# RemyMuj/UnityRayTracer

Measured on AMD Instinct MI355X. Metric: Mrays/sec @1920x1080, 8 bounces, higher is better.
Workload: dtype f32

## Files before the change

### include/urt_math.h

```cpp
#pragma once
#include <stdint.h>

#if defined(__HIPCC__)
#include <hip/hip_runtime.h>
#define URT_HD __host__ __device__ __forceinline__
#else
#define URT_HD inline __attribute__((always_inline))
#endif

#if defined(__clang__)
#pragma clang fp contract(off)
#endif

namespace urt {

static constexpr float kPI        = 3.14159265f;
static constexpr float kEPSILON   = 1e-8f;
static constexpr float kFLOAT_MAX = 3.402823466e+38f;
#define URT_INF (__builtin_inff())

URT_HD float f_fma(float a, float b, float c) { return __builtin_fmaf(a, b, c); }
URT_HD float f_sqrt(float x) { return __builtin_sqrtf(x); }
URT_HD float f_floor(float x) { return __builtin_floorf(x); }
URT_HD float f_abs(float x) { return __builtin_fabsf(x); }
// ... 189 lines not shown
  }
}
URT_HD void cslab(float cx, float cy, float cz, float hx, float hy, float hz, const CRay& R, float tbest, float& tn, float& tf) {
  float mx = f_fma(cx, R.idir.x, R.b.x), my = f_fma(cy, R.idir.y, R.b.y), mz = f_fma(cz, R.idir.z, R.b.z);
  float dx = f_fma(hx, f_abs(R.idir.x), R.pa.x), dy = f_fma(hy, f_abs(R.idir.y), R.pa.y), dz = f_fma(hz, f_abs(R.idir.z), R.pa.z);
  tn = f_max(f_max(f_max(mx - dx, my - dy), mz - dz), 0.0f);
  tf = f_min(f_min(f_min(mx + dx, my + dy), mz + dz), tbest);
}

URT_HD bool tlas_cull(float t_min, float t_max, float t_ground) {
  const float kappa = 0.015625f;
  float s = kappa * (f_abs(t_min) + f_abs(t_max));
  bool miss = (t_min - t_max) > s;
  bool behind = t_max < -s;
  bool beyond = (t_min - t_ground) > kappa * (f_abs(t_min) + f_abs(t_ground));
  return miss || behind || beyond;
}

URT_HD float f_div_const(float x, float c, float y) {
  float ax = f_abs(x);
  if (!(ax >= 1e-30f && ax <= 3.0e38f)) return x / c;
  float q = x * y;
  float r = f_fma(-q, c, x);
  return f_fma(r, y, q);
}

URT_HD float rand_next(float& seed, float px, float py) {
  float a = f_div_const(seed + f_div_const(seed, 17.0f, 1.0f / 17.0f), 100.0f, 1.0f / 100.0f);
  float d = dot2(px, py, 12.9898f, 78.233f);
  float r = f_frac(f_sin(a * d) * 43758.5453f);
  seed = seed + 0.5f;
  return r;
}

}
```

### unityraytracer_amd/csrc/context_impl.h

```cpp
#pragma once
#include <hip/hip_runtime.h>

#include <algorithm>
#include <cmath>
#include <cstdio>
#include <cstring>
#include <new>
#include <string>
#include <unordered_map>
#include <utility>
#include <vector>

#include "../../include/urt.h"
#include "../../include/urt_math.h"
#include "blas_builder.h"
#include "kernels.h"
#include "owned.h"
#include "urt_device.h"

namespace urtd {

struct Buffer {
  int count = 0, stride = 0;
  std::vector<uint8_t> host;
// ... 120 lines not shown
    int32_t* d_mesh_leaf = nullptr;
    size_t cap_mesh_leaf = 0;
    int walk_f4 = 0;
    int n_blas_nodes = 0;
    int n_scene_tris = 0;
    int scene_max_depth = 0;
    int tlas_stack = 2, blas_stack = 2;
    unsigned int watchdog_steps = 1u << 16;
    std::vector<int32_t> h_mesh_root, h_small_first;
    std::vector<int32_t> h_vert_lo, h_vert_hi;
    int n_vertices = 0, n_normals = 0;
    std::vector<float> h_cost_base;
    std::vector<uint8_t> prev_mesh_objects;
  } scene;
  uint64_t scene_epoch = 0;
  float last_prepare_ms = 0;
  int last_builder = 0;
  uint64_t refitted_meshes = 0, incremental_preps = 0;
  uint64_t deformed_meshes = 0, renormed_meshes = 0, deform_bytes = 0, forced_rebuilds = 0;
  float last_cost_ratio = 0;
  urtd::BlasCache blas_cache;
  int sched_groups = 0;
  urtd::DeviceBuf<float4> zero_sky;

  urtd::PathQueues q{};
  urtd::DeviceBuf<float4> q_store[2][4];
  urtd::DeviceBuf<unsigned int> q_counts;

  urtd::DeviceBuf<urtd::DevCounters> d_counters;
  static constexpr size_t kStampOffset = urtd::kWorkShards * 128, kStampBytes = 65536 * 16 * sizeof(unsigned long long), kWorkCounterBytes = kStampOffset + kStampBytes;
  urtd::DeviceBuf<unsigned int> d_next;
  urtd::DeviceBuf<float4> d_mail;
  static constexpr int kTableSlots = 4;
  urtd::PinnedBuf<urtd::FrameUniforms> h_tables; urtd::DeviceBuf<urtd::FrameUniforms> d_tables;
  urtd::Event table_ev[kTableSlots];
  unsigned int table_next = 0;
  uint64_t pixels_dispatched = 0;
  int n_cus = 256;

  uint64_t dispatches = 0;
  std::vector<std::pair<urtd::Event, urtd::Event>> timing;
  float trace_ms = 0;

  enum class OpKind { BlendAdd, BlendHistory, Copy, PackRows };
  struct PostOp {
    OpKind kind;
    int frame;
    urt_handle src = 0, dst = 0;
    float sample = 0;
    urt_handle count = 0; float max_history = 0;
    void* dense = nullptr; int first_row = 0, row_stride = 1; bool rgb = false;
    bool touches(urt_handle t) const { return src == t || dst == t || count == t; }
  };
  struct Pending {
    int n = 0, limit = 1;
    urt_handle tex = 0;
    uint64_t scene_epoch = 0;
    urtd::DevScene S{};
    urtd::FrameParams P{};
    urtd::FrameTable T{};
    int front_mode = 0; bool count = false;
    std::vector<PostOp> ops;
  } pend;
  urtd::DeviceBuf<float4> slab;
  size_t slab_stride = 0;
  int slab_frames = 0;
  urt_handle slab_tex = 0;
// ... 120 lines not shown
```

### unityraytracer_amd/csrc/experiments.h

```cpp
#pragma once

#if defined(URT_STAMPS) || defined(URT_SCHED_OCC) || defined(URT_SERVE_OCC) || defined(URT_SERVE_SLEEP) || defined(URT_SKY_FASTWRAP) || \
    defined(URT_SAH_BINS) || defined(URT_AB)
#ifndef URT_EXPERIMENT
#error "A/B, probe and diagnostic switches (-DURT_STAMPS, -DURT_SCHED_OCC, -DURT_SAH_BINS, ...) need -DURT_EXPERIMENT: the library then reports a negative urt_abi_version and loaders refuse it unless they opt in (csrc/experiments.h)"
#endif
#endif

#ifdef URT_EXPERIMENT
#define URT_ABI_SIGN (-1)
#else
#define URT_ABI_SIGN 1
#endif
```

### unityraytracer_amd/csrc/frame_batch.cpp

```cpp
#include "experiments.h"
#include "context_impl.h"

#include "reproject.h"

namespace urtd {

static unsigned int sched_trip_cap(urt_context* ctx, const FrameParams& P, int n_frames) {
  if (ctx->opt.watchdog_cap > 0) return (unsigned int)ctx->opt.watchdog_cap;
  uint64_t per = std::max<uint64_t>(1, (uint64_t)std::max(1, P.num_rays) * (uint64_t)std::max(1, P.num_bounces) / 8u);
  uint64_t cap = (1ull << 24) * (uint64_t)std::max(1, n_frames) * per;
  return (unsigned int)std::min<uint64_t>(cap, 0xfffffff0ull);
}

static int ensure_queues(urt_context* ctx, size_t n_paths, size_t n_counts) {
  for (int k = 0; k < 8; k++) {
    if (int rc = reserve(ctx, ctx->q_store[k / 4][k % 4], n_paths, "path queue allocation", touch(ctx))) return rc;
    ctx->q.s[k / 4][k % 4] = ctx->q_store[k / 4][k % 4].get();
  }
  if (int rc = reserve(ctx, ctx->q_counts, n_counts, "path queue allocation", touch(ctx))) return rc;
  ctx->q.counts = ctx->q_counts.get();
  return URT_OK;
}

int resolve_timing(urt_context* ctx) {
// ... 157 lines not shown

template <typename Launch>
static int timed_launch(urt_context* ctx, hipStream_t st, int kernel_mode, int front_mode, const FrameParams& P, bool count, int waves_per_cu, Launch launch) {
  Event e0, e1;
  if (ctx->opt.time_dispatch) {
    int rc = take_event(ctx, &e0); if (rc) return rc;
    rc = take_event(ctx, &e1); if (rc) return rc;
    URT_HIP(ctx, hipEventRecord(e0.get(), st));
  }
  TraceLaunchRecord rec{};
  hipError_t le = launch(&rec);
  if (ctx->opt.time_dispatch) {
    (void)hipEventRecord(e1.get(), st);
    ctx->timing.emplace_back(std::move(e0), std::move(e1));
  }
  ctx->launches++;
  if (le != hipSuccess) return fail(ctx, URT_ERR_HIP, std::string("kernel launch: ") + hipGetErrorString(le));
  record_launch(ctx, rec, kernel_mode, front_mode, P, count, waves_per_cu);
  return URT_OK;
}

static constexpr int kAutoFrames = 64;

static int launch_sched_frames(urt_context* ctx, const DevScene& S, const FrameParams& P, const FrameTable& T, float4* result,
                        int front_mode, bool count, hipStream_t st = nullptr, unsigned int* next = nullptr) {
  if (!st) { st = touch(ctx); next = ctx->d_next.get(); }
  if (!ctx->h_tables) {
    URT_HIP(ctx, ctx->h_tables.alloc((size_t)kMaxFramesPerLaunch * urt_context::kTableSlots));
    URT_HIP(ctx, ctx->d_tables.alloc((size_t)kMaxFramesPerLaunch * urt_context::kTableSlots));
    for (Event& ev : ctx->table_ev) URT_HIP(ctx, ev.create(hipEventDisableTiming));
  }
  const unsigned int slot = ctx->table_next++ % (unsigned int)urt_context::kTableSlots;
  if (ctx->table_next > (unsigned int)urt_context::kTableSlots) URT_HIP(ctx, hipEventSynchronize(ctx->table_ev[slot].get()));
  FrameUniforms* h_slot = ctx->h_tables.get() + (size_t)slot * kMaxFramesPerLaunch;
  FrameUniforms* d_table = ctx->d_tables.get() + (size_t)slot * kMaxFramesPerLaunch;
  std::memcpy(h_slot, T.f, sizeof(FrameUniforms) * (size_t)P.n_frames);
  URT_HIP(ctx, hipMemcpyAsync(d_table, h_slot, sizeof(FrameUniforms) * (size_t)P.n_frames, hipMemcpyHostToDevice, st));
  URT_HIP(ctx, hipEventRecord(ctx->table_ev[slot].get(), st));
  int waves_per_block = P.block_threads / 64;
  long want = ((long)P.tiles_x * P.n_strips * P.n_frames + waves_per_block - 1) / waves_per_block;
  int wpc = ctx->opt.waves_per_cu;
  if (wpc <= 0) wpc = P.serve ? 16 : 20;
  if (ctx->sched_groups > 0) wpc = ctx->sched_groups * waves_per_block;
  long resident = (long)ctx->n_cus * wpc / waves_per_block;
  int nb = (int)std::max(1L, std::min(want, resident));
  if (P.serve) {
    if (int rc = reserve(ctx, ctx->d_mail, (size_t)nb * (size_t)P.block_threads * 2, "mailbox allocation", touch(ctx))) return rc;
  }
  int rc = timed_launch(ctx, st, P.serve ? 5 : 3, front_mode, P, count, wpc, [&](TraceLaunchRecord* rec) {
    return P.serve ? launch_serve(S, P, d_table, result, ctx->d_counters.get(), next, ctx->d_mail.get(), nb, front_mode, count, st, rec)
                   : launch_sched(S, P, d_table, result, ctx->d_counters.get(), next, nb, front_mode, count, st, rec);
  });
  if (rc == URT_OK) ctx->last_launch.cones = !P.serve && !count && !S.blas_qnodes && S.blas_cnodes && ctx->scene.cones_in_use ? 1 : 0;
  return rc;
}

struct BlendRun { int frames; urt_handle present; size_t end; };
static BlendRun blend_run(const std::vector<PostOp>& ops, size_t i, urt_handle result_tex, float* samples) {
  const PostOp& op = ops[i];
  size_t j = i, j_present = i;
  int cnt = 0, cnt_present = 0;
  urt_handle present = 0;
  while (j < ops.size() && cnt <= kMaxFramesPerLaunch) {
    const PostOp& q = ops[j];
    if (q.kind == op.kind && q.dst == op.dst && q.count == op.count && q.max_history == op.max_history && q.frame == op.frame + cnt &&
        cnt < kMaxFramesPerLaunch) { samples[cnt++] = q.sample; j++; }
    else if (q.kind == OpKind::Copy && q.src == op.dst && q.dst != op.dst && q.dst != op.count && q.dst != result_tex && (present == 0 || q.dst == present)) {
      present = q.dst; j++; j_present = j; cnt_present = cnt;
    } else break;
  }
// ... 193 lines not shown
  if ((mode == 3 || mode == 5) && P.num_bounces >= (1 << 24)) mode = 2;
  bool count = ctx->opt.count_stats != 0;
  const int region[4] = {P.region_w, P.region_h, first_row, row_stride};
  const bool full_cover = P.region_w == res->w && P.region_h == res->h && first_row == 0 && row_stride == 1;

  if (mode == 3 || mode == 5) {
    bool top_in_front = ctx->opt.top_front < 0 ? S.n_meshes > 1 : ctx->opt.top_front != 0;
    P.serve = mode == 5 && ctx->scene.n_blas_nodes > 0;
    P.pool_inloop = ctx->opt.serve_refill;
    int front_mode = configure_sched(ctx, S, P, top_in_front);
    P.shade_split = ctx->opt.shade_split != 0;
    set_handout(ctx, P);
    P.front_fuse = ctx->opt.front_fuse == 0 ? 0 : (S.n_mesh_tlas == 1 && S.n_meshes > 0 && S.n_spheres == 0 ? 2 : 1);
    const FrameUniforms fu = bound_camera(ctx);
    bool same_region = res->n_regions == 1 && std::memcmp(res->rg, region, sizeof region) == 0;
    bool renamable = !res->external && !res->ptr_exposed && (full_cover || (!res->other_writes && (res->n_regions == 0 || same_region)));
    int limit = renamable ? batch_limit(ctx, P) : 1;
    urt_context::Pending& B = ctx->pend;
    if (B.n > 0) {
      const FrameParams& Q = B.P;
      bool same = B.tex == res_h && B.scene_epoch == ctx->scene_epoch && B.S.sky == S.sky && B.S.sky_w == S.sky_w && B.S.sky_h == S.sky_h &&
                  B.count == count && B.front_mode == front_mode && Q.serve == P.serve && Q.num_bounces == P.num_bounces && Q.num_rays == P.num_rays &&
                  Q.width == P.width && Q.height == P.height && Q.region_w == P.region_w && Q.region_h == P.region_h &&
                  Q.first_group_row == P.first_group_row && Q.row_stride == P.row_stride && B.n < B.limit && limit > 1;
      if (!same) { int rc = flush_pending(ctx); if (rc) return rc; }
    }
    if (limit > 1 && B.n == 0) {
      int rc = ensure_slab(ctx, res_h, *res, limit); if (rc) return rc;
      if (!ctx->slab || ctx->slab_tex != res_h || ctx->slab_frames < 2) limit = 1;
    }
    if (B.n == 0) { int rc = bind_sky(ctx, S); if (rc) return rc; }
    if (limit <= 1) {
      FrameTable T{};
      T.f[0] = fu;
      P.frame_group = 1;
      int rc = launch_sched_frames(ctx, S, P, T, res->dev, front_mode, count);
      if (rc) return rc;
    } else {
      if (B.n == 0) {
        B.limit = std::min(limit, ctx->slab_frames);
        B.tex = res_h; B.scene_epoch = ctx->scene_epoch; B.S = S; B.P = P; B.front_mode = front_mode; B.count = count;
      }
      B.T.f[B.n] = fu;
      res->dev = ctx->slab.get() + (size_t)B.n * ctx->slab_stride;
      B.n++;
    }
  } else {
    int rc = flush_pending(ctx); if (rc) return rc;
    int nb = 0, k = 0;
    if (mode == 1) {
      size_t n_paths = (size_t)P.tiles_x * 64 * (size_t)P.n_strips;
      rc = ensure_queues(ctx, n_paths, (size_t)P.num_rays * (size_t)(P.num_bounces + 1));
      if (rc) return rc;
    } else if (mode == 2) {
      int waves_per_block = P.block_threads / 64;
      long want = ((long)P.tiles_x * P.n_strips + waves_per_block - 1) / waves_per_block;
      int wpc = ctx->opt.waves_per_cu;
      if (wpc <= 0) wpc = 20;
      long resident = (long)ctx->n_cus * wpc / waves_per_block;
      nb = (int)std::max(1L, std::min(want, resident));
    } else if (mode == 4) {
      P.block_threads = 64;
      P.refill_min = ctx->opt.pool_refill; P.blas_min = ctx->opt.pool_blas_min; P.blas_exit = ctx->opt.pool_blas_exit;
      P.pool_inloop = ctx->opt.pool_inloop; P.pool_other_min = ctx->opt.pool_other_min;
      k = ctx->opt.pool_k;
      size_t lds = pool_lds_bytes(P, k);
      while (k > 1 && lds > 160 * 1024) { k--; lds = pool_lds_bytes(P, k); }
      if (lds > 160 * 1024) return fail(ctx, URT_ERR_OUT_OF_MEMORY, "kernel_mode 4: the scene's traversal stacks do not fit the LDS of one CU; use kernel_mode 3");
      int fit = (int)std::max<size_t>(1, (160 * 1024) / lds);
      int wpc = ctx->opt.waves_per_cu > 0 ? ctx->opt.waves_per_cu : fit;
      long want = ((long)P.tiles_x * P.n_strips * 64 + 64L * k - 1) / (64L * k);
      nb = (int)std::max(1L, std::min(want, (long)ctx->n_cus * wpc));
    }
    const hipStream_t st = touch(ctx);
    rc = timed_launch(ctx, st, mode, 0, P, count, ctx->opt.waves_per_cu, [&](TraceLaunchRecord* rec) {
      switch (mode) {
// ... 15 lines not shown
```

### unityraytracer_amd/csrc/frame_device.h

```cpp
#pragma once
#include <hip/hip_runtime.h>
#include <stdint.h>

#include "../../include/urt_math.h"
#include "urt_device.h"
#include "kernels.h"

using namespace urt;
using namespace urtd;

#include "camera_device.h"
#include "trace_device.h"
#include "sky_device.h"
#include "shade_device.h"

namespace {

template <bool COUNT>
__device__ __forceinline__ HitRec trace(const DevScene& S, v3 o, v3 d, int* tl, int* bl, LocalCounters& lc) {
  return trace_ray<COUNT, false>(S, o, d, URT_INF, tl, bl, lc);
}

typedef const __attribute__((address_space(4))) float* kfloatp;
__device__ __forceinline__ kfloatp kernarg_floats(unsigned byte_offset) {
  const __attribute__((address_space(4))) char* p = (const __attribute__((address_space(4))) char*)__builtin_amdgcn_kernarg_segment_ptr();
  p += byte_offset;
  asm volatile("" : "+s"(p));
  return (kfloatp)p;
}

template <unsigned P_OFF>
__device__ __forceinline__ void camera_ray(const FrameParams& P, int x, int y, float& seed, v3& o, v3& d) {
  float u, v;
  jitter_uv(seed, (float)x, (float)y, P.pixel_off_x, P.pixel_off_y, P.width, P.height, u, v);
  kfloatp c2w = kernarg_floats(P_OFF + (unsigned)__builtin_offsetof(FrameParams, c2w));
  kfloatp invp = kernarg_floats(P_OFF + (unsigned)__builtin_offsetof(FrameParams, invp));
  camera_ray_uv(c2w, invp, u, v, o, d);
}
__device__ __forceinline__ void camera_ray_frame(const FrameUniforms* T, int f, const FrameParams& P, int x, int y, bool new_pixel, float& seed, v3& o, v3& d) {
  kfloatp q = (kfloatp)(unsigned long long)(T + __builtin_amdgcn_readfirstlane(f));
  if (new_pixel) seed = q[34];
  float px = (float)x, py = (float)y;
  float r0 = rand_next(seed, px, py);
  float r1 = rand_next(seed, px, py);
  float u = axis_uv(px + r0 + q[32], P.width);
  float v = axis_uv(py + r1 + q[33], P.height);
  camera_ray_uv(q, q + 16, u, v, o, d);
}
static_assert(__builtin_offsetof(FrameUniforms, invp) == 64 && __builtin_offsetof(FrameUniforms, pixel_off_x) == 128 &&
              __builtin_offsetof(FrameUniforms, seed) == 136, "camera_ray_frame indexes the table as floats");

template <typename F>
__device__ __forceinline__ void for_each_frame(bool pred, int frame, F&& body) {
  unsigned long long todo = wballot(pred);
  while (todo) {
    int f = __builtin_amdgcn_readlane(frame, __builtin_ctzll(todo));
    bool mine = pred && frame == f;
    body(f, mine);
    todo &= ~wballot(mine);
  }
}

static constexpr unsigned kPOffAfterScene = (unsigned)((sizeof(DevScene) + alignof(FrameParams) - 1) / alignof(FrameParams) * alignof(FrameParams));

__device__ __forceinline__ bool tile_pixel(const FrameParams& P, int& x, int& y) {
  int wave = threadIdx.x >> 6, lane = threadIdx.x & 63;
  int b = blockIdx.x;
  int G = P.xcd_run;
  int sb = ((b / (8 * G)) * 8 + (b & 7)) * G + ((b >> 3) % G);
  int tile = sb * (blockDim.x >> 6) + wave;
  int ntiles = P.tiles_x * P.n_strips;
  if (tile >= ntiles) return false;
  int ty = tile / P.tiles_x, tx = tile - ty * P.tiles_x;
  x = tx * 8 + (lane & 7);
  y = (P.first_group_row + ty * P.row_stride) * 8 + (lane >> 3);
  return x < P.region_w && y < P.region_h;
}

__device__ __forceinline__ unsigned int wave_sum(unsigned int v) {
  for (int off = 32; off > 0; off >>= 1) v += __shfl_xor(v, off, 64);
  return v;
}

// ... 139 lines not shown
    }
  }
  return run_word(nshard, f, t0, vt * 64u, exh);
}

__device__ __forceinline__ bool wg_fetch_pixels(const FrameParams& P, unsigned long long want, bool mine, unsigned int* next,
                                                unsigned int ntiles, unsigned long long* rs, bool& exhausted, int& x, int& y,
                                                unsigned int tiles_per_frame, int* frame, unsigned long long* n_adds = nullptr) {
  const int lane = threadIdx.x & 63;
  const unsigned int n = (unsigned int)__popcll(want);
  const unsigned int rank = (unsigned int)__popcll(want & ((1ull << lane) - 1ull));
  unsigned int taken = 0;
  bool got = false;
  for (int round = 0; round < 2; round++) {
    unsigned long long s = 0;
    unsigned int k = 0, avail = 0;
    bool fetch = false;
    for (int tries = 0;; tries++) {
      if (tries == kRunCasTries) return got;
      s = wave_uniform64(__hip_atomic_load(rs, __ATOMIC_RELAXED, __HIP_MEMORY_SCOPE_WORKGROUP));
      avail = ((unsigned int)(s >> 11) & 0x7ffu) - ((unsigned int)s & 0x7ffu);
      unsigned long long s2;
      if (avail) {
        k = min(n - taken, avail);
        fetch = k == avail && !(s & kRunExhausted);
        s2 = (s + k) | (fetch ? kRunFetching : 0ull);
      } else if (s & kRunExhausted) { exhausted = true; return got; }
      else if (s & kRunFetching) { if (n == 64u) __builtin_amdgcn_s_sleep(2); return got; }
      else { k = 0; fetch = true; s2 = s | kRunFetching; }
      unsigned long long seen = s;
      if (lane == 0) __hip_atomic_compare_exchange_strong(rs, &seen, s2, __ATOMIC_RELAXED, __ATOMIC_RELAXED, __HIP_MEMORY_SCOPE_WORKGROUP);
      if (wave_uniform64(seen) == s) break;
    }
    if (mine && rank >= taken && rank < taken + k) {
      const unsigned int idx = ((unsigned int)s & 0x7ffu) + (rank - taken);
      unsigned int tile = ((unsigned int)(s >> 24) & 0xffffffu) + (idx >> 6), f = (unsigned int)(s >> 48) & 0x7fu;
      if (tile >= tiles_per_frame) { unsigned int q = tile / tiles_per_frame; f += q; tile -= q * tiles_per_frame; }
      *frame = (int)f;
      if (P.tile_order == 1) tile = tiles_per_frame - 1u - tile;
      got = slot_pixel(P, tile, idx & 63u, x, y);
    }
    taken += k;
    if (!fetch) { if (k == avail) exhausted = true; break; }
    const unsigned long long ns = wg_fetch_run(P, (unsigned int)(s >> 55) & 63u, next, ntiles, tiles_per_frame);
    if (lane == 0) __hip_atomic_store(rs, ns, __ATOMIC_RELAXED, __HIP_MEMORY_SCOPE_WORKGROUP);
    if (n_adds) ++*n_adds;
    if (taken == n) break;
  }
  return got;
}

__device__ __forceinline__ void report_watchdog(const FrameParams& P, DevCounters* shard) {
  atomicAdd(&shard->watchdog, 1ull);
  if (P.trip_flag) __hip_atomic_fetch_add(P.trip_flag, 1u, __ATOMIC_RELAXED, __HIP_MEMORY_SCOPE_SYSTEM);
}

__device__ __forceinline__ void finish_path(const FrameParams& P, float4* result, int pixel, int ray_index, v3 res, float seed) {
  int x = pixel & 0xffff, y = (unsigned)pixel >> 16;
  size_t at = (size_t)y * P.width + x;
  v3 avg = res;
  if (ray_index > 0) { float4 prev = result[at]; avg = xyz(prev) + res; }
  if (ray_index == P.num_rays - 1) {
    float n = (float)P.num_rays;
    result[at] = make_float4(avg.x / n, avg.y / n, avg.z / n, 1.0f);
  } else {
    result[at] = make_float4(avg.x, avg.y, avg.z, seed);
  }
}

}
```

### unityraytracer_amd/csrc/kernels.h

```cpp
#pragma once
#include <hip/hip_runtime.h>
#include "urt_device.h"

namespace urtd {

struct TraceLaunchRecord { char kernel[96]; int n_blocks, block_threads, lds_bytes; };

hipError_t launch_mega(const DevScene& S, const FrameParams& P, float4* result, DevCounters* ctr, bool count, hipStream_t st, TraceLaunchRecord* rec);
hipError_t launch_wavefront(const DevScene& S, const FrameParams& P, const PathQueues& Q, float4* result, DevCounters* ctr,
                            bool count, hipStream_t st, TraceLaunchRecord* rec);
hipError_t launch_persist(const DevScene& S, const FrameParams& P, float4* result, DevCounters* ctr, unsigned int* next,
                          int n_blocks, bool count, hipStream_t st, TraceLaunchRecord* rec);
hipError_t launch_sched(const DevScene& S, const FrameParams& P, const FrameUniforms* T, float4* result, DevCounters* ctr,
                        unsigned int* next, int n_blocks, int front_mode, bool count, hipStream_t st, TraceLaunchRecord* rec);
hipError_t launch_serve(const DevScene& S, const FrameParams& P, const FrameUniforms* T, float4* result, DevCounters* ctr,
                        unsigned int* next, float4* mail, int n_blocks, int front_mode, bool count, hipStream_t st, TraceLaunchRecord* rec);
hipError_t launch_blit_add_multi(const float4* src, size_t frame_stride, int n, const float* samples, float4* dst, float4* present,
                                 size_t n_pixels, hipStream_t st);
size_t sched_lds_bytes(const DevScene& S, const FrameParams& P);
hipError_t launch_pool(const DevScene& S, const FrameParams& P, float4* result, DevCounters* ctr, unsigned int* next,
                       int n_blocks, int k, bool count, hipStream_t st, TraceLaunchRecord* rec);
size_t pool_lds_bytes(const FrameParams& P, int k);
hipError_t launch_blit_add(const float4* src, float4* dst, size_t n_pixels, float sample, hipStream_t st);
hipError_t launch_pack_rows(float4* img, float4* dense, int width, int height, int first_group_row, int row_stride,
                            int n_strips, bool to_dense, hipStream_t st);

hipError_t launch_pack_rows_rgb(float4* img, float* dense, int width, int height, int first_group_row, int row_stride,
                                int n_strips, bool to_dense, float alpha, hipStream_t st);

}
```

### unityraytracer_amd/csrc/kernels.hip

```cpp
#include "experiments.h"
#include "front_device.h"
#include "launch_host.h"
#include <utility>

namespace {

#ifndef URT_SCHED_OCC
#define URT_SCHED_OCC 5
#endif
template <bool COUNT, int BLOCK, int FMODE, bool MULTI, bool QN = false>
__global__ __launch_bounds__(BLOCK, URT_SCHED_OCC) void k_sched(DevScene S, FrameParams P, const FrameUniforms* __restrict__ T, float4* __restrict__ result, DevCounters* ctr,
                                               unsigned int* __restrict__ next) {
  constexpr bool CONES = !COUNT && !QN;
  extern __shared__ int lds[];
  float4* lds4 = (float4*)lds;
  const float4* top = lds4 + 1;
  if (threadIdx.x == 0) *(unsigned long long*)lds = run_word(blockIdx.x & ((unsigned int)P.n_shards - 1u), 0, 0, 0, false);
  for (int i = threadIdx.x; i < P.top_nodes * 4; i += blockDim.x) lds4[1 + i] = S.blas_cnodes[i];
  int at = 1 + P.top_nodes * 4;
  FrontLds L;
  if (P.lds_mesh) {
    for (int i = threadIdx.x; i < 2 * S.n_mesh_tlas; i += blockDim.x) lds4[at + i] = S.mesh_tlas[i];
    L.mesh_tlas = lds4 + at; at += 2 * S.n_mesh_tlas;
    for (int i = threadIdx.x; i < S.n_meshes; i += blockDim.x) ((int32_t*)(lds4 + at))[i] = S.mesh_root[i];
    L.mesh_root = (const int32_t*)(lds4 + at); at += (S.n_meshes + 3) / 4;
    if (P.lds_small) {
      for (int i = threadIdx.x; i < S.n_meshes; i += blockDim.x) ((int32_t*)(lds4 + at))[i] = S.mesh_small_first[i];
      L.small_first = (const int32_t*)(lds4 + at); at += (S.n_meshes + 3) / 4;
      for (int m = threadIdx.x; m < S.n_meshes; m += blockDim.x) {
        int sf = S.mesh_small_first[m];
        if (sf >= 0) {
          uint32_t code = ~(uint32_t)S.mesh_root[m];
          uint32_t first = code >> 3, cnt = (code & 7u) + 1u;
          for (uint32_t q = 0; q < 3 * cnt; q++) lds4[at + 3 * sf + q] = S.tri_verts[3 * (size_t)first + q];
        }
      }
      L.small_tris = lds4 + at; at += 3 * S.n_small;
    }
  }
  WalkLds W;
  if (FMODE == 3) {
    const float4* wsrc = S.mesh_tlas + 2 * S.n_mesh_tlas;
    for (int i = threadIdx.x; i < P.walk_f4; i += blockDim.x) lds4[at + i] = wsrc[i];
    W.hdr = (const int*)(lds4 + at); W.pos_tab = W.hdr + 16; W.eval = lds4 + at + 20; at += P.walk_f4;
// ... 316 lines not shown
  size_t per_strip = (size_t)width * 8;
  size_t n = per_strip * (size_t)n_strips;
  for (size_t i = (size_t)blockIdx.x * blockDim.x + threadIdx.x; i < n; i += (size_t)gridDim.x * blockDim.x) {
    int j = (int)(i / per_strip);
    size_t r = i - (size_t)j * per_strip;
    int row = (first_group_row + j * row_stride) * 8 + (int)(r / (size_t)width);
    int col = (int)(r % (size_t)width);
    float* d = dense + 3 * i;
    if (row < height) {
      size_t at = (size_t)row * width + col;
      if (to_dense) { float4 v = img[at]; d[0] = v.x; d[1] = v.y; d[2] = v.z; }
      else const_cast<float4*>(img)[at] = make_float4(d[0], d[1], d[2], alpha);
    } else if (to_dense) {
      d[0] = 0; d[1] = 0; d[2] = 0;
    }
  }
}

}

namespace urtd {

size_t sched_lds_bytes(const DevScene& S, const FrameParams& P) {
  size_t f4 = (size_t)P.top_nodes * 4;
  if (P.lds_mesh) f4 += 2 * (size_t)S.n_mesh_tlas + ((size_t)S.n_meshes + 3) / 4;
  if (P.walk_f4 > 0) f4 += (size_t)P.walk_f4 + (P.lds_small ? 3 * (size_t)S.n_small : 0);
  else if (P.lds_small) f4 += ((size_t)S.n_meshes + 3) / 4 + 3 * (size_t)S.n_small;
  if (P.lds_sphere) f4 += 2 * (size_t)S.n_sphere_tlas + (size_t)S.n_spheres;
  if (P.serve) f4 += 2 * (size_t)P.block_threads + 1;
  else f4 += 1;
  return f4 * 16 + (size_t)(P.tlas_stack + P.blas_stack) * 64 * (size_t)(P.block_threads / 64) * sizeof(int);
}

using SchedKernel = void (*)(DevScene, FrameParams, const FrameUniforms*, float4*, DevCounters*, unsigned int*);
template <int I>
static constexpr SchedKernel sched_entry() {
  constexpr bool COUNT = (I & 1) != 0, MULTI = (I & 2) != 0, QN = (I & 4) != 0;
  if constexpr (COUNT && QN) return nullptr;
  else return k_sched<COUNT, (I & 32) ? 256 : 64, (I >> 3) & 3, MULTI, QN>;
}
template <int... I>
static SchedKernel sched_kernel(bool count, int block, int fmode, bool multi, bool qn, std::integer_sequence<int, I...>) {
  static const SchedKernel table[] = {sched_entry<I>()...};
  return table[(count ? 1 : 0) | (multi ? 2 : 0) | (qn ? 4 : 0) | (fmode << 3) | (block == 256 ? 32 : 0)];
}

hipError_t launch_sched(const DevScene& S, const FrameParams& P, const FrameUniforms* T, float4* result, DevCounters* ctr,
                        unsigned int* next, int n_blocks, int front_mode, bool count, hipStream_t st, TraceLaunchRecord* rec) {
  if (n_blocks <= 0) return hipSuccess;
  if (P.block_threads != 64 && P.block_threads != 256) return hipErrorInvalidValue;
  if (!batched_args_ok(S, P, front_mode)) return hipErrorInvalidValue;
  if (front_mode == 3 && (P.walk_f4 < 20 || P.lds_mesh || P.top_nodes <= 0 || S.n_mesh_tlas > 31)) return hipErrorInvalidValue;
  if (front_mode != 3 && P.walk_f4 != 0) return hipErrorInvalidValue;
  hipError_t e = reset_work_counters(next, st);
  if (e != hipSuccess) return e;
  const int block = P.block_threads;
  const int fmode = front_mode < 1 || front_mode > 3 || (front_mode == 1 && P.top_nodes <= 0) ? 0 : front_mode;
  const bool multi = P.num_rays > 1, qn = !count && S.blas_qnodes;
  return launch_traced(named(rec, "k_sched<%s, %d, %d, %s, %s>", tf(count), block, fmode, tf(multi), tf(qn)),
                       sched_kernel(count, block, fmode, multi, qn, std::make_integer_sequence<int, 64>()),
                       n_blocks, block, sched_lds_bytes(S, P), st, S, P, T, result, ctr, next);
}

hipError_t launch_blit_add(const float4* src, float4* dst, size_t n_pixels, float sample, hipStream_t st) {
  if (n_pixels == 0) return hipSuccess;
  size_t nb = (n_pixels + 255) / 256;
  if (nb > 2048) nb = 2048;
  hipLaunchKernelGGL(k_blit_add, dim3((unsigned)nb), dim3(256), 0, st, src, dst, n_pixels, sample);
  return hipGetLastError();
}

hipError_t launch_blit_add_multi(const float4* src, size_t frame_stride, int n, const float* samples, float4* dst, float4* present,
                                 size_t n_pixels, hipStream_t st) {
  if (n_pixels == 0 || n <= 0) return hipSuccess;
  if (n > kMaxFramesPerLaunch) return hipErrorInvalidValue;
  BlendSamples smp{};
  for (int f = 0; f < n; f++) smp.s[f] = samples[f];
  size_t nb = (n_pixels + 255) / 256;
  if (nb > 4096) nb = 4096;
  hipLaunchKernelGGL(k_blit_add_multi, dim3((unsigned)nb), dim3(256), 0, st, src, frame_stride, n, smp, dst, present, n_pixels);
// ... 27 lines not shown
```

### unityraytracer_amd/csrc/kernels_serve.hip

```cpp
#include "experiments.h"
#include "front_device.h"
#include "launch_host.h"

namespace {

enum : int { ST_WAIT = 6 };
enum : int { MB_IDLE = 0, MB_REQ = 1, MB_BUSY = 2, MB_DONE = 3 };

__device__ __forceinline__ int lanes_below(unsigned long long m) {
  return (int)__builtin_amdgcn_mbcnt_hi((unsigned int)(m >> 32), __builtin_amdgcn_mbcnt_lo((unsigned int)m, 0u));
}
__device__ __forceinline__ int lds_load(const int* p) { return __hip_atomic_load(p, __ATOMIC_RELAXED, __HIP_MEMORY_SCOPE_WORKGROUP); }
__device__ __forceinline__ void lds_store(int* p, int v) { __hip_atomic_store(p, v, __ATOMIC_RELAXED, __HIP_MEMORY_SCOPE_WORKGROUP); }

#ifndef URT_SERVE_OCC
#define URT_SERVE_OCC 4
#endif
#ifndef URT_SERVE_SLEEP
#define URT_SERVE_SLEEP 8
#endif
__device__ __forceinline__ void serve_wait(bool waiting, const int* my_flag, const int* avail) {
  for (int spin = 0; spin < 64; spin++) {
    __builtin_amdgcn_s_sleep(URT_SERVE_SLEEP);
    bool done = waiting && (lds_load(my_flag) & 3) == MB_DONE;
    if (wballot(done) != 0 || __builtin_amdgcn_readfirstlane(lds_load(avail)) > 0) break;
  }
}
template <bool COUNT, int BLOCK, int FMODE, bool MULTI>
__global__ __launch_bounds__(BLOCK, URT_SERVE_OCC) void k_serve(DevScene S, FrameParams P, const FrameUniforms* __restrict__ T, float4* __restrict__ result, DevCounters* ctr,
                                               unsigned int* __restrict__ next, float4* __restrict__ mail) {
  constexpr int NW = BLOCK / 64;
  static_assert(NW >= 1 && (NW & (NW - 1)) == 0, "waves per workgroup: a power of two");
  extern __shared__ int lds[];
  float4* lds4 = (float4*)lds;
  const float4* top = lds4;
  for (int i = threadIdx.x; i < P.top_nodes * 4; i += blockDim.x) lds4[i] = S.blas_cnodes[i];
  int at = P.top_nodes * 4;
  FrontLds L;
  if (P.lds_mesh) {
    for (int i = threadIdx.x; i < 2 * S.n_mesh_tlas; i += blockDim.x) lds4[at + i] = S.mesh_tlas[i];
    L.mesh_tlas = lds4 + at; at += 2 * S.n_mesh_tlas;
    for (int i = threadIdx.x; i < S.n_meshes; i += blockDim.x) ((int32_t*)(lds4 + at))[i] = S.mesh_root[i];
    L.mesh_root = (const int32_t*)(lds4 + at); at += (S.n_meshes + 3) / 4;
    if (P.lds_small) {
      for (int i = threadIdx.x; i < S.n_meshes; i += blockDim.x) ((int32_t*)(lds4 + at))[i] = S.mesh_small_first[i];
      L.small_first = (const int32_t*)(lds4 + at); at += (S.n_meshes + 3) / 4;
      for (int m = threadIdx.x; m < S.n_meshes; m += blockDim.x) {
        int sf = S.mesh_small_first[m];
        if (sf >= 0) {
          uint32_t code = ~(uint32_t)S.mesh_root[m];
          uint32_t first = code >> 3, cnt = (code & 7u) + 1u;
          for (uint32_t q = 0; q < 3 * cnt; q++) lds4[at + 3 * sf + q] = S.tri_verts[3 * (size_t)first + q];
        }
      }
      L.small_tris = lds4 + at; at += 3 * S.n_small;
    }
  }
  if (P.lds_sphere) {
    for (int i = threadIdx.x; i < 2 * S.n_sphere_tlas; i += blockDim.x) lds4[at + i] = S.sphere_tlas[i];
    L.sphere_tlas = lds4 + at; at += 2 * S.n_sphere_tlas;
    for (int i = threadIdx.x; i < S.n_spheres; i += blockDim.x) lds4[at + i] = S.sphere_pr[i];
    L.sphere_pr = lds4 + at; at += S.n_spheres;
// ... 241 lines not shown
          v3 sum = (MULTI ? avg : mk3(0, 0, 0)) + res;
          if (MULTI) { avg = sum; ray_i++; next_ray = ray_i < P.num_rays; }
          if (!next_ray) {
            float n = (float)P.num_rays;
            st_nt(result + (size_t)((unsigned)kf >> 24) * P.frame_stride + (size_t)((unsigned)xy >> 16) * P.width + (xy & 0xffff),
                      MULTI ? make_float4(sum.x / n, sum.y / n, sum.z / n, 1.0f) : make_float4(sum.x, sum.y, sum.z, 1.0f));
            st = ST_DEAD;
          }
        }
      }
      if (MULTI) {
        for_each_frame(next_ray, (int)((unsigned)kf >> 24), [&](int f, bool mine) {
          if (mine) {
            res = mk3(0, 0, 0); energy = mk3(1, 1, 1); kf &= (int)0xff000000;
            camera_ray_frame(T, f, P, xy & 0xffff, (int)((unsigned)xy >> 16), false, seed, o, d);
          }
        });
      }
    }
  }
  if (watchdog && (threadIdx.x & 63) == 0) report_watchdog(P, ctr);
  if (COUNT && (threadIdx.x & 63) == 0) {
    DevCounters* c = ctr + (blockIdx.x & (kCounterShards - 1));
    for (int q = 0; q < 6; q++) if (sv[q]) atomicAdd(&c->serve[q], sv[q]);
  }
  lc.rays = (threadIdx.x & 63) == 0 ? wave_rays : 0u;
  flush_counters<COUNT>(lc, ctr);
}

}

namespace urtd {

using ServeKernel = void (*)(DevScene, FrameParams, const FrameUniforms*, float4*, DevCounters*, unsigned int*, float4*);
template <bool COUNT, bool MULTI>
static ServeKernel serve_kernel_f(int fmode) {
  return fmode == 2 ? k_serve<COUNT, 256, 2, MULTI> : fmode == 1 ? k_serve<COUNT, 256, 1, MULTI> : k_serve<COUNT, 256, 0, MULTI>;
}
static ServeKernel serve_kernel(bool count, int fmode, bool multi) {
  return count ? (multi ? serve_kernel_f<true, true>(fmode) : serve_kernel_f<true, false>(fmode))
               : (multi ? serve_kernel_f<false, true>(fmode) : serve_kernel_f<false, false>(fmode));
}

hipError_t launch_serve(const DevScene& S, const FrameParams& P, const FrameUniforms* T, float4* result, DevCounters* ctr,
                        unsigned int* next, float4* mail, int n_blocks, int front_mode, bool count, hipStream_t st, TraceLaunchRecord* rec) {
  if (n_blocks <= 0) return hipSuccess;
  if (P.block_threads != 256 || !P.serve || !mail) return hipErrorInvalidValue;
  if (!batched_args_ok(S, P, front_mode)) return hipErrorInvalidValue;
  hipError_t e = reset_work_counters(next, st);
  if (e != hipSuccess) return e;
  const int fmode = front_mode < 1 || front_mode > 2 || (front_mode == 1 && P.top_nodes <= 0) ? 0 : front_mode;
  const bool multi = P.num_rays > 1;
  return launch_traced(named(rec, "k_serve<%s, 256, %d, %s>", tf(count), fmode, tf(multi)), serve_kernel(count, fmode, multi), n_blocks, 256,
                       sched_lds_bytes(S, P), st, S, P, T, result, ctr, next, mail);
}

}
```

### unityraytracer_amd/csrc/urt_device.h

```cpp
#pragma once
#include <stdint.h>
#include <hip/hip_runtime.h>

#include "blas_builder.h"

namespace urtd {

struct DevScene {
  const float4* mesh_tlas;   int n_mesh_tlas;
  const float4* sphere_tlas; int n_sphere_tlas;
  const float4* sphere_pr;   int n_spheres;
  const float4* materials;
  const int32_t* mesh_root;  int n_meshes;
  const int32_t* mesh_small_first; int n_small;
  const float4* blas_nodes;
  const float4* blas_cnodes;
  const float4* blas_qnodes;
  const float4* tri_verts;
  const float4* tri_norms;
  const float4* sky;         int sky_w, sky_h;
  int cull_any;
};

struct FrameParams {
  float c2w[16];
  float invp[16];
  float pixel_off_x, pixel_off_y;
  float seed;
  int num_bounces;
  int num_rays;
  int width, height;
  int region_w, region_h;
  int tiles_x;
  int first_group_row;
  int row_stride;
  int n_strips;
  int tlas_stack;
// ... 6 lines not shown
  int refill_min;
  int blas_min;
  int shade_min;
  int sky_min;
  int shade_split;
  int blas_exit;
  int top_nodes;
  int lds_small;
  int lds_mesh, lds_sphere;
  int walk_f4;
  int serve;
  union {
    int pool_inloop;
    int handout;
  };
  union {
    int pool_other_min;
    int front_fuse;
  };
  unsigned int watchdog_steps;
  unsigned int sched_trips;
  unsigned int* trip_flag;
  int n_frames;
  unsigned int frame_stride;
};

struct FrameUniforms {
  float c2w[16];
  float invp[16];
  float pixel_off_x, pixel_off_y;
  float seed;
  float pad;
};
static constexpr int kMaxFramesPerLaunch = 64;
struct FrameTable { FrameUniforms f[kMaxFramesPerLaunch]; };

struct LaneStackSize { int tlas, blas; };

static constexpr unsigned int kWorkShards = 64;
static constexpr int kCounterShards = 256;
struct alignas(128) DevCounters {
  unsigned long long rays, tlas_nodes, blas_nodes, tri_tests, sphere_tests;
  unsigned long long hit_tri, hit_sphere, hit_ground, hit_sky;
  unsigned long long watchdog;
  unsigned long long serve[6];
};
static_assert(sizeof(DevCounters) == 128, "one counter shard = one 128-byte line");

struct PathQueues {
  float4* s[2][4];
  unsigned int* counts;
};

}
```

Measured before the change: 21030.

## Precompute per-frame RNG scales and camera origin on host for camera ray refill

Extends the per-frame table with host-computed RNG scale factors and the camera origin, so the device camera-ray path for a new pixel uses them directly instead of recomputing the seed-derived divisions and the origin transform per lane. The refill pixel-assignment loop is also restructured to iterate over tiles uniformly across the wave, doing wave-uniform tile decoding rather than per-lane divergent decoding. This trades a larger frame table entry and a loop over tiles for less per-ray arithmetic and divergence at refill time.

```diff
diff --git a/include/urt_math.h b/include/urt_math.h
--- a/include/urt_math.h
+++ b/include/urt_math.h
@@ -245,5 +245,12 @@
   seed = seed + 0.5f;
   return r;
 }
-
-}
+URT_HD float rand_scale(float seed) {
+  return f_div_const(seed + f_div_const(seed, 17.0f, 1.0f / 17.0f), 100.0f, 1.0f / 100.0f);
+}
+URT_HD float rand_draw(float a, float px, float py) {
+  float d = dot2(px, py, 12.9898f, 78.233f);
+  return f_frac(f_sin(a * d) * 43758.5453f);
+}
+
+}
diff --git a/unityraytracer_amd/csrc/context_impl.h b/unityraytracer_amd/csrc/context_impl.h
--- a/unityraytracer_amd/csrc/context_impl.h
+++ b/unityraytracer_amd/csrc/context_impl.h
@@ -176,7 +176,7 @@
   urtd::DeviceBuf<unsigned int> d_next;
   urtd::DeviceBuf<float4> d_mail;
   static constexpr int kTableSlots = 4;
-  urtd::PinnedBuf<urtd::FrameUniforms> h_tables; urtd::DeviceBuf<urtd::FrameUniforms> d_tables;
+  urtd::PinnedBuf<urtd::FrameEntry> h_tables; urtd::DeviceBuf<urtd::FrameEntry> d_tables;
   urtd::Event table_ev[kTableSlots];
   unsigned int table_next = 0;
   uint64_t pixels_dispatched = 0;
diff --git a/unityraytracer_amd/csrc/experiments.h b/unityraytracer_amd/csrc/experiments.h
--- a/unityraytracer_amd/csrc/experiments.h
+++ b/unityraytracer_amd/csrc/experiments.h
@@ -1,6 +1,6 @@
 #pragma once
 
-#if defined(URT_STAMPS) || defined(URT_SCHED_OCC) || defined(URT_SERVE_OCC) || defined(URT_SERVE_SLEEP) || defined(URT_SKY_FASTWRAP) || \
+#if defined(URT_STAMPS) || defined(URT_SCHED_OCC) || defined(URT_SERVE_OCC) || defined(URT_SERVE_SLEEP) || defined(URT_SKY_FASTWRAP) || defined(URT_UNIFORM_REFILL) || \
     defined(URT_SAH_BINS) || defined(URT_AB)
 #ifndef URT_EXPERIMENT
 #error "A/B, probe and diagnostic switches (-DURT_STAMPS, -DURT_SCHED_OCC, -DURT_SAH_BINS, ...) need -DURT_EXPERIMENT: the library then reports a negative urt_abi_version and loaders refuse it unless they opt in (csrc/experiments.h)"
diff --git a/unityraytracer_amd/csrc/frame_batch.cpp b/unityraytracer_amd/csrc/frame_batch.cpp
--- a/unityraytracer_amd/csrc/frame_batch.cpp
+++ b/unityraytracer_amd/csrc/frame_batch.cpp
@@ -213,10 +213,10 @@
   }
   const unsigned int slot = ctx->table_next++ % (unsigned int)urt_context::kTableSlots;
   if (ctx->table_next > (unsigned int)urt_context::kTableSlots) URT_HIP(ctx, hipEventSynchronize(ctx->table_ev[slot].get()));
-  FrameUniforms* h_slot = ctx->h_tables.get() + (size_t)slot * kMaxFramesPerLaunch;
-  FrameUniforms* d_table = ctx->d_tables.get() + (size_t)slot * kMaxFramesPerLaunch;
-  std::memcpy(h_slot, T.f, sizeof(FrameUniforms) * (size_t)P.n_frames);
-  URT_HIP(ctx, hipMemcpyAsync(d_table, h_slot, sizeof(FrameUniforms) * (size_t)P.n_frames, hipMemcpyHostToDevice, st));
+  FrameEntry* h_slot = ctx->h_tables.get() + (size_t)slot * kMaxFramesPerLaunch;
+  FrameEntry* d_table = ctx->d_tables.get() + (size_t)slot * kMaxFramesPerLaunch;
+  std::memcpy(h_slot, T.f, sizeof(FrameEntry) * (size_t)P.n_frames);
+  URT_HIP(ctx, hipMemcpyAsync(d_table, h_slot, sizeof(FrameEntry) * (size_t)P.n_frames, hipMemcpyHostToDevice, st));
   URT_HIP(ctx, hipEventRecord(ctx->table_ev[slot].get(), st));
   int waves_per_block = P.block_threads / 64;
   long want = ((long)P.tiles_x * P.n_strips * P.n_frames + waves_per_block - 1) / waves_per_block;
@@ -476,7 +476,7 @@
     if (B.n == 0) { int rc = bind_sky(ctx, S); if (rc) return rc; }
     if (limit <= 1) {
       FrameTable T{};
-      T.f[0] = fu;
+      T.f[0] = frame_entry(fu);
       P.frame_group = 1;
       int rc = launch_sched_frames(ctx, S, P, T, res->dev, front_mode, count);
       if (rc) return rc;
@@ -485,7 +485,7 @@
         B.limit = std::min(limit, ctx->slab_frames);
         B.tex = res_h; B.scene_epoch = ctx->scene_epoch; B.S = S; B.P = P; B.front_mode = front_mode; B.count = count;
       }
-      B.T.f[B.n] = fu;
+      B.T.f[B.n] = frame_entry(fu);
       res->dev = ctx->slab.get() + (size_t)B.n * ctx->slab_stride;
       B.n++;
     }
diff --git a/unityraytracer_amd/csrc/frame_derived.h b/unityraytracer_amd/csrc/frame_derived.h
--- /dev/null
+++ b/unityraytracer_amd/csrc/frame_derived.h
@@ -0,0 +1,21 @@
+#pragma once
+#include "../../include/urt_math.h"
+
+namespace urtd {
+
+struct FrameDerived {
+  float a0;
+  float a1;
+  float origin[3];
+};
+
+inline FrameDerived frame_derived(const float* c2w, float seed) {
+  FrameDerived d;
+  d.a0 = urt::rand_scale(seed);
+  d.a1 = urt::rand_scale(seed + 0.5f);
+  const urt::v3 o = urt::mul_m4(c2w, 0.0f, 0.0f, 0.0f, 1.0f);
+  d.origin[0] = o.x; d.origin[1] = o.y; d.origin[2] = o.z;
+  return d;
+}
+
+}
diff --git a/unityraytracer_amd/csrc/frame_device.h b/unityraytracer_amd/csrc/frame_device.h
--- a/unityraytracer_amd/csrc/frame_device.h
+++ b/unityraytracer_amd/csrc/frame_device.h
@@ -37,10 +37,25 @@
   kfloatp invp = kernarg_floats(P_OFF + (unsigned)__builtin_offsetof(FrameParams, invp));
   camera_ray_uv(c2w, invp, u, v, o, d);
 }
-__device__ __forceinline__ void camera_ray_frame(const FrameUniforms* T, int f, const FrameParams& P, int x, int y, bool new_pixel, float& seed, v3& o, v3& d) {
+#ifndef URT_UNIFORM_REFILL
+#define URT_UNIFORM_REFILL 1
+#endif
+__device__ __forceinline__ void camera_ray_frame(const FrameEntry* T, int f, const FrameParams& P, int x, int y, bool new_pixel, float& seed, v3& o, v3& d) {
   kfloatp q = (kfloatp)(unsigned long long)(T + __builtin_amdgcn_readfirstlane(f));
+  float px = (float)x, py = (float)y;
+  if (URT_UNIFORM_REFILL && new_pixel) {
+    float r0 = rand_draw(q[36], px, py);
+    float r1 = rand_draw(q[37], px, py);
+    seed = (q[34] + 0.5f) + 0.5f;
+    float u = axis_uv(px + r0 + q[32], P.width);
+    float v = axis_uv(py + r1 + q[33], P.height);
+    v3 dir = mul_m4_k(q + 16, u, v, 0.0f, 1.0f);
+    dir = mul_m4_k(q, dir.x, dir.y, dir.z, 0.0f);
+    o = mk3(q[38], q[39], q[40]);
+    d = normalize(dir);
+    return;
+  }
   if (new_pixel) seed = q[34];
-  float px = (float)x, py = (float)y;
   float r0 = rand_next(seed, px, py);
   float r1 = rand_next(seed, px, py);
   float u = axis_uv(px + r0 + q[32], P.width);
@@ -48,7 +63,8 @@
   camera_ray_uv(q, q + 16, u, v, o, d);
 }
 static_assert(__builtin_offsetof(FrameUniforms, invp) == 64 && __builtin_offsetof(FrameUniforms, pixel_off_x) == 128 &&
-              __builtin_offsetof(FrameUniforms, seed) == 136, "camera_ray_frame indexes the table as floats");
+              __builtin_offsetof(FrameUniforms, seed) == 136 && __builtin_offsetof(FrameEntry, d) == 144 && __builtin_offsetof(FrameDerived, a1) == 4 &&
+              __builtin_offsetof(FrameDerived, origin) == 8 && sizeof(FrameEntry) == 164, "camera_ray_frame indexes the table as floats");
 
 template <typename F>
 __device__ __forceinline__ void for_each_frame(bool pred, int frame, F&& body) {
@@ -254,6 +270,26 @@
       if (lane == 0) __hip_atomic_compare_exchange_strong(rs, &seen, s2, __ATOMIC_RELAXED, __ATOMIC_RELAXED, __HIP_MEMORY_SCOPE_WORKGROUP);
       if (wave_uniform64(seen) == s) break;
     }
+#if URT_UNIFORM_REFILL
+    if (k) {
+      const unsigned int first = (unsigned int)s & 0x7ffu;
+      const unsigned int idx = first + (rank - taken);
+      const bool in = mine && rank >= taken && rank < taken + k;
+      for (unsigned int t = first >> 6; t <= (first + k - 1u) >> 6; t++) {
+        unsigned int tile = ((unsigned int)(s >> 24) & 0xffffffu) + t, f = (unsigned int)(s >> 48) & 0x7fu;
+        if (tile >= tiles_per_frame) { unsigned int q = tile / tiles_per_frame; f += q; tile -= q * tiles_per_frame; }
+        if (P.tile_order == 1) tile = tiles_per_frame - 1u - tile;
+        const int ty = (int)tile / P.tiles_x, tx = (int)tile - ty * P.tiles_x;
+        const int x0 = tx * 8, y0 = (P.first_group_row + ty * P.row_stride) * 8;
+        if (in && (idx >> 6) == t) {
+          *frame = (int)f;
+          x = x0 + (int)(idx & 7u);
+          y = y0 + (int)((idx >> 3) & 7u);
+          got = x < P.region_w && y < P.region_h;
+        }
+      }
+    }
+#else
     if (mine && rank >= taken && rank < taken + k) {
       const unsigned int idx = ((unsigned int)s & 0x7ffu) + (rank - taken);
       unsigned int tile = ((unsigned int)(s >> 24) & 0xffffffu) + (idx >> 6), f = (unsigned int)(s >> 48) & 0x7fu;
@@ -262,6 +298,7 @@
       if (P.tile_order == 1) tile = tiles_per_frame - 1u - tile;
       got = slot_pixel(P, tile, idx & 63u, x, y);
     }
+#endif
     taken += k;
     if (!fetch) { if (k == avail) exhausted = true; break; }
     const unsigned long long ns = wg_fetch_run(P, (unsigned int)(s >> 55) & 63u, next, ntiles, tiles_per_frame);
diff --git a/unityraytracer_amd/csrc/kernels.h b/unityraytracer_amd/csrc/kernels.h
--- a/unityraytracer_amd/csrc/kernels.h
+++ b/unityraytracer_amd/csrc/kernels.h
@@ -11,9 +11,9 @@
                             bool count, hipStream_t st, TraceLaunchRecord* rec);
 hipError_t launch_persist(const DevScene& S, const FrameParams& P, float4* result, DevCounters* ctr, unsigned int* next,
                           int n_blocks, bool count, hipStream_t st, TraceLaunchRecord* rec);
-hipError_t launch_sched(const DevScene& S, const FrameParams& P, const FrameUniforms* T, float4* result, DevCounters* ctr,
+hipError_t launch_sched(const DevScene& S, const FrameParams& P, const FrameEntry* T, float4* result, DevCounters* ctr,
                         unsigned int* next, int n_blocks, int front_mode, bool count, hipStream_t st, TraceLaunchRecord* rec);
-hipError_t launch_serve(const DevScene& S, const FrameParams& P, const FrameUniforms* T, float4* result, DevCounters* ctr,
+hipError_t launch_serve(const DevScene& S, const FrameParams& P, const FrameEntry* T, float4* result, DevCounters* ctr,
                         unsigned int* next, float4* mail, int n_blocks, int front_mode, bool count, hipStream_t st, TraceLaunchRecord* rec);
 hipError_t launch_blit_add_multi(const float4* src, size_t frame_stride, int n, const float* samples, float4* dst, float4* present,
                                  size_t n_pixels, hipStream_t st);
diff --git a/unityraytracer_amd/csrc/kernels.hip b/unityraytracer_amd/csrc/kernels.hip
--- a/unityraytracer_amd/csrc/kernels.hip
+++ b/unityraytracer_amd/csrc/kernels.hip
@@ -9,7 +9,7 @@
 #define URT_SCHED_OCC 5
 #endif
 template <bool COUNT, int BLOCK, int FMODE, bool MULTI, bool QN = false>
-__global__ __launch_bounds__(BLOCK, URT_SCHED_OCC) void k_sched(DevScene S, FrameParams P, const FrameUniforms* __restrict__ T, float4* __restrict__ result, DevCounters* ctr,
+__global__ __launch_bounds__(BLOCK, URT_SCHED_OCC) void k_sched(DevScene S, FrameParams P, const FrameEntry* __restrict__ T, float4* __restrict__ result, DevCounters* ctr,
                                                unsigned int* __restrict__ next) {
   constexpr bool CONES = !COUNT && !QN;
   extern __shared__ int lds[];
@@ -392,7 +392,7 @@
   return f4 * 16 + (size_t)(P.tlas_stack + P.blas_stack) * 64 * (size_t)(P.block_threads / 64) * sizeof(int);
 }
 
-using SchedKernel = void (*)(DevScene, FrameParams, const FrameUniforms*, float4*, DevCounters*, unsigned int*);
+using SchedKernel = void (*)(DevScene, FrameParams, const FrameEntry*, float4*, DevCounters*, unsigned int*);
 template <int I>
 static constexpr SchedKernel sched_entry() {
   constexpr bool COUNT = (I & 1) != 0, MULTI = (I & 2) != 0, QN = (I & 4) != 0;
@@ -405,7 +405,7 @@
   return table[(count ? 1 : 0) | (multi ? 2 : 0) | (qn ? 4 : 0) | (fmode << 3) | (block == 256 ? 32 : 0)];
 }
 
-hipError_t launch_sched(const DevScene& S, const FrameParams& P, const FrameUniforms* T, float4* result, DevCounters* ctr,
+hipError_t launch_sched(const DevScene& S, const FrameParams& P, const FrameEntry* T, float4* result, DevCounters* ctr,
                         unsigned int* next, int n_blocks, int front_mode, bool count, hipStream_t st, TraceLaunchRecord* rec) {
   if (n_blocks <= 0) return hipSuccess;
   if (P.block_threads != 64 && P.block_threads != 256) return hipErrorInvalidValue;
diff --git a/unityraytracer_amd/csrc/kernels_serve.hip b/unityraytracer_amd/csrc/kernels_serve.hip
--- a/unityraytracer_amd/csrc/kernels_serve.hip
+++ b/unityraytracer_amd/csrc/kernels_serve.hip
@@ -27,7 +27,7 @@
   }
 }
 template <bool COUNT, int BLOCK, int FMODE, bool MULTI>
-__global__ __launch_bounds__(BLOCK, URT_SERVE_OCC) void k_serve(DevScene S, FrameParams P, const FrameUniforms* __restrict__ T, float4* __restrict__ result, DevCounters* ctr,
+__global__ __launch_bounds__(BLOCK, URT_SERVE_OCC) void k_serve(DevScene S, FrameParams P, const FrameEntry* __restrict__ T, float4* __restrict__ result, DevCounters* ctr,
                                                unsigned int* __restrict__ next, float4* __restrict__ mail) {
   constexpr int NW = BLOCK / 64;
   static_assert(NW >= 1 && (NW & (NW - 1)) == 0, "waves per workgroup: a power of two");
@@ -335,7 +335,7 @@
 
 namespace urtd {
 
-using ServeKernel = void (*)(DevScene, FrameParams, const FrameUniforms*, float4*, DevCounters*, unsigned int*, float4*);
+using ServeKernel = void (*)(DevScene, FrameParams, const FrameEntry*, float4*, DevCounters*, unsigned int*, float4*);
 template <bool COUNT, bool MULTI>
 static ServeKernel serve_kernel_f(int fmode) {
   return fmode == 2 ? k_serve<COUNT, 256, 2, MULTI> : fmode == 1 ? k_serve<COUNT, 256, 1, MULTI> : k_serve<COUNT, 256, 0, MULTI>;
@@ -345,7 +345,7 @@
                : (multi ? serve_kernel_f<false, true>(fmode) : serve_kernel_f<false, false>(fmode));
 }
 
-hipError_t launch_serve(const DevScene& S, const FrameParams& P, const FrameUniforms* T, float4* result, DevCounters* ctr,
+hipError_t launch_serve(const DevScene& S, const FrameParams& P, const FrameEntry* T, float4* result, DevCounters* ctr,
                         unsigned int* next, float4* mail, int n_blocks, int front_mode, bool count, hipStream_t st, TraceLaunchRecord* rec) {
   if (n_blocks <= 0) return hipSuccess;
   if (P.block_threads != 256 || !P.serve || !mail) return hipErrorInvalidValue;
diff --git a/unityraytracer_amd/csrc/urt_device.h b/unityraytracer_amd/csrc/urt_device.h
--- a/unityraytracer_amd/csrc/urt_device.h
+++ b/unityraytracer_amd/csrc/urt_device.h
@@ -3,6 +3,7 @@
 #include <hip/hip_runtime.h>
 
 #include "blas_builder.h"
+#include "frame_derived.h"
 
 namespace urtd {
 
@@ -75,8 +76,13 @@
   float seed;
   float pad;
 };
+struct FrameEntry {
+  FrameUniforms u;
+  FrameDerived d;
+};
+inline FrameEntry frame_entry(const FrameUniforms& u) { return FrameEntry{u, frame_derived(u.c2w, u.seed)}; }
 static constexpr int kMaxFramesPerLaunch = 64;
-struct FrameTable { FrameUniforms f[kMaxFramesPerLaunch]; };
+struct FrameTable { FrameEntry f[kMaxFramesPerLaunch]; };
 
 struct LaneStackSize { int tlas, blas; };
 
```

Measured after the change: 21320, median of 6. +1.4%, better.
